# BioinformaticsToolsmith/MeShClust

Measured on AMD Instinct MI355X. Metric: sequences clustered/sec (+ NW cell-updates/sec) at 1/2/4/8 MI355X, higher is better.
Workload: dtype u8

## Files before the change

### include/meshclust_amd.h

```cpp
#ifndef MESHCLUST_AMD_H
#define MESHCLUST_AMD_H

#include <stddef.h>
#include <stdint.h>

#ifdef __cplusplus
extern "C" {
#endif

#define MC_ABI_VERSION 1

#define MC_OK 0
#define MC_ERR_ARG 1
#define MC_ERR_HIP 2
#define MC_ERR_STATE 3
#define MC_ERR_OOM 4
#define MC_ERR_INPUT 5
#define MC_ERR_UNSUPPORTED 6
#define MC_ERR_TIMEOUT 7

#define MC_FEAT_ALIGN (1 << 0)
#define MC_FEAT_LD (1 << 1)
#define MC_FEAT_MANHATTAN (1 << 2)
#define MC_FEAT_INTERSECTION (1 << 4)
// ... 86 lines not shown
int mc_orient_pairs(mc_ctx *ctx, const uint32_t *a, const uint32_t *b, uint64_t m, uint8_t *strand ,
                    uint64_t *sad );

#define MC_ASSIGN_MAX_TOP 8
int mc_assign_top(mc_ctx *ctx, const uint32_t *centre_ids, uint32_t C, const uint32_t *query_ids, uint64_t M,
                  double sim, int strands , uint32_t K ,
                  uint32_t *hit , double *hit_val , uint8_t *hit_strand ,
                  uint32_t *n_similar , uint64_t *stats );

int mc_nw_identity(mc_ctx *ctx, const uint32_t *a, const uint32_t *b, uint64_t m, double *ident,
                   int32_t *len, int32_t *ids);

int mc_nw_identity_raw(mc_ctx *ctx, const uint8_t *a, const uint64_t *a_off, const uint8_t *b,
                       const uint64_t *b_off, uint64_t m, double *ident, int32_t *len,
                       int32_t *ids, int32_t *score);

int mc_revcomp_sequences(mc_ctx *ctx, const uint32_t *ids, uint64_t m, uint8_t *bytes, uint64_t *off);

#define MC_IDENT_BATCH_PAIRS (1ull << 20)
#define MC_IDENT_BATCH_BYTES (256ull << 20)
int mc_nw_identity_strands(mc_ctx *ctx, const uint32_t *a, const uint32_t *b, const uint8_t *a_minus, uint64_t m,
                           double *ident, int32_t *len, int32_t *ids);

#define MC_CIGAR_I 1u
#define MC_CIGAR_D 2u
#define MC_CIGAR_EQ 7u
#define MC_CIGAR_X 8u
#define MC_ALIGN_BATCH_PAIRS (1ull << 16)
#define MC_ALIGN_SCRATCH_BYTES (1ull << 30)
int mc_nw_align_strands(mc_ctx *ctx, const uint32_t *a, const uint32_t *b, const uint8_t *a_minus, uint64_t m,
                        uint32_t *cigar, uint64_t cap, uint64_t *cig_off ,
                        int32_t *score, int32_t *len, int32_t *ids);
int mc_nw_align_profile(mc_ctx *ctx, double *out , int reset);

int mc_set_align_band(mc_ctx *ctx, int mode );
int mc_nw_band_plan(mc_ctx *ctx, const uint32_t *a, const uint32_t *b, const uint8_t *a_minus, uint64_t m,
                    int32_t *w , int32_t *score );
int mc_nw_band_profile(mc_ctx *ctx, double *out , int reset);

#define MC_PILEUP_CH 8
int mc_nw_pileup_strands(mc_ctx *ctx, const uint32_t *a, const uint32_t *b, const uint8_t *a_minus, uint64_t m,
                         const uint32_t *targets, uint32_t nt, uint64_t *row_off ,
                         uint32_t *table , uint64_t cap_rows,
                         int32_t *score, int32_t *len, int32_t *ids );
int mc_nw_pileup_profile(mc_ctx *ctx, double *out , int reset);

// ... 89 lines not shown
```

### meshclust_amd/__init__.py

```python
import ctypes as C
import os
import subprocess

import numpy as np

HERE = os.path.dirname(os.path.abspath(__file__))
ROOT = os.path.dirname(HERE)
LIB_DIR = os.path.join(HERE, "lib")
BIN = os.path.join(HERE, "bin", "meshclust")
GPU_LIB = os.environ.get("MC_GPU_LIB", os.path.join(LIB_DIR, "libmcgpu.so"))
HOST_LIB = os.path.join(LIB_DIR, "libmeshclust.so")
HEADER = os.path.join(ROOT, "include", "meshclust_amd.h")

FEAT_ALIGN, FEAT_LD, FEAT_MANHATTAN = 1, 2, 4
FEAT_INTERSECTION, FEAT_PEARSON, FEAT_KULCZYNSKI2 = 16, 32, 1024
COMBO_SQUARED, COMBO_SELF = 1, 2
ASSIGN_NONE = 0xFFFFFFFF
MC_STRAND_PLUS, MC_STRAND_MINUS = 1, 2
ASSIGN_MAX_TOP = 8
ERR_ARG, ERR_UNSUPPORTED = 1, 6
ERR_STATE = 3
CIGAR_I, CIGAR_D, CIGAR_EQ, CIGAR_X = 1, 2, 7, 8
PILEUP_CH = 8
MSA_GAP = ord("-")
MSA_CH = 8
QUAL_MAX = 93
FAMILIES = ("kmer", "keys", "pairs", "scan", "finalize", "mean_shift", "nw", "layout")


class MCError(RuntimeError):
    pass


def build(jobs=8):
    subprocess.run(["make", "-s", "-j%d" % jobs, "-C", os.path.join(HERE, "csrc")], check=True)


class Classifier(C.Structure):
    _fields_ = [
        ("n_single", C.c_int32),
        ("lookup", C.c_uint16 * 8),
        ("is_sim", C.c_int32 * 8),
        ("mins", C.c_double * 8),
        ("maxs", C.c_double * 8),
        ("n_combo", C.c_int32),
        ("combo_kind", C.c_int32 * 8),
        ("combo_len", C.c_int32 * 8),
        ("combo_idx", (C.c_int32 * 4) * 8),
        ("weights", C.c_double * 9),
# ... 19 lines not shown


def _p(a):
    return a.ctypes.data_as(C.c_void_p) if a is not None else None


def gpu_lib():
    global _gpu
    if _gpu is None:
        if not os.path.exists(GPU_LIB):
            raise ImportError("libmcgpu.so not built (run meshclust_amd.build()); no CPU fallback exists")
        lib = C.CDLL(GPU_LIB)
        lib.mc_last_error.restype = C.c_char_p
        lib.mc_ctx_create.argtypes = [C.c_int, C.POINTER(C.c_void_p)]
        lib.mc_ctx_destroy.argtypes = [C.c_void_p]
        for name in ("mc_load_sequences", "mc_load_packed", "mc_kmer_max", "mc_kmer_build", "mc_get_histograms", "mc_distance_keys",
                     "mc_pair_features", "mc_set_classifier", "mc_classify_pairs", "mc_nw_identity",
                     "mc_nw_identity_raw", "mc_set_order", "mc_kill", "mc_cluster_begin", "mc_scan",
                     "mc_mean_shift", "mc_update_iteration", "mc_timers", "mc_classify_values", "mc_mean_shift_select", "mc_accumulate",
                     "mc_scan_part", "mc_scan_commit", "mc_comm_unique_id", "mc_comm_create", "mc_comm_allgather",
                     "mc_comm_stats", "mc_comm_destroy", "mc_sync", "mc_assign", "mc_assign_strands",
                     "mc_revcomp_rows", "mc_assign_top", "mc_revcomp_sequences", "mc_nw_identity_strands",
                     "mc_nw_align_strands", "mc_nw_align_profile", "mc_nw_pileup_strands", "mc_nw_pileup_profile",
                     "mc_kmer_max_strands", "mc_kmer_build_strands", "mc_orient_pairs"):
            getattr(lib, name).restype = C.c_int
        lib.mc_comm_create.argtypes = [C.c_int, C.c_int, C.c_int, C.c_char_p, C.POINTER(C.c_void_p)]
        lib.mc_comm_allgather.argtypes = [C.c_void_p, C.c_void_p, C.c_uint64, C.c_void_p]
        lib.mc_comm_stats.argtypes = [C.c_void_p, C.POINTER(C.c_uint64), C.POINTER(C.c_uint64)]
        lib.mc_comm_destroy.argtypes = [C.c_void_p, C.c_int]
        lib.mc_assign.argtypes = [C.c_void_p, C.c_void_p, C.c_uint32, C.c_void_p, C.c_uint64, C.c_double,
                                  C.c_void_p, C.c_void_p, C.c_void_p, C.c_void_p]
        lib.mc_assign_strands.argtypes = [C.c_void_p, C.c_void_p, C.c_uint32, C.c_void_p, C.c_uint64, C.c_double, C.c_int,
                                          C.c_void_p, C.c_void_p, C.c_void_p, C.c_void_p, C.c_void_p]
        lib.mc_revcomp_rows.argtypes = [C.c_void_p, C.c_void_p, C.c_uint64, C.c_void_p]
        lib.mc_assign_top.argtypes = [C.c_void_p, C.c_void_p, C.c_uint32, C.c_void_p, C.c_uint64, C.c_double, C.c_int,
                                      C.c_uint32, C.c_void_p, C.c_void_p, C.c_void_p, C.c_void_p, C.c_void_p]
        lib.mc_revcomp_sequences.argtypes = [C.c_void_p, C.c_void_p, C.c_uint64, C.c_void_p, C.c_void_p]
        lib.mc_nw_identity_strands.argtypes = [C.c_void_p, C.c_void_p, C.c_void_p, C.c_void_p, C.c_uint64, C.c_void_p,
                                               C.c_void_p, C.c_void_p]
        lib.mc_nw_align_strands.argtypes = [C.c_void_p, C.c_void_p, C.c_void_p, C.c_void_p, C.c_uint64, C.c_void_p,
                                            C.c_uint64, C.c_void_p, C.c_void_p, C.c_void_p, C.c_void_p]
        lib.mc_nw_align_profile.argtypes = [C.c_void_p, C.c_void_p, C.c_int]
        lib.mc_nw_pileup_strands.argtypes = [C.c_void_p, C.c_void_p, C.c_void_p, C.c_void_p, C.c_uint64, C.c_void_p, C.c_uint32,
                                             C.c_void_p, C.c_void_p, C.c_uint64, C.c_void_p, C.c_void_p, C.c_void_p]
        lib.mc_nw_pileup_profile.argtypes = [C.c_void_p, C.c_void_p, C.c_int]
        lib.mc_kmer_max_strands.argtypes = [C.c_void_p, C.c_int, C.c_int, C.POINTER(C.c_uint64)]
        lib.mc_kmer_build_strands.argtypes = [C.c_void_p, C.c_int, C.c_int, C.c_int]
        lib.mc_orient_pairs.argtypes = [C.c_void_p, C.c_void_p, C.c_void_p, C.c_uint64, C.c_void_p, C.c_void_p]
        lib.mc_load_qualities.restype = C.c_int
        lib.mc_load_qualities.argtypes = [C.c_void_p, C.c_void_p, C.c_uint64]
        lib.mc_nw_qpileup_strands.restype = C.c_int
        lib.mc_nw_qpileup_strands.argtypes = [C.c_void_p, C.c_void_p, C.c_void_p, C.c_void_p, C.c_uint64, C.c_void_p, C.c_uint32,
                                              C.c_void_p, C.c_void_p, C.c_void_p, C.c_uint64, C.c_void_p, C.c_void_p, C.c_void_p]
        for name in ("mc_nw_msa_begin", "mc_nw_msa_rows", "mc_nw_msa_end", "mc_nw_msa_profile"):
            getattr(lib, name).restype = C.c_int
        lib.mc_nw_msa_begin.argtypes = [C.c_void_p, C.c_void_p, C.c_void_p, C.c_void_p, C.c_uint64, C.c_void_p, C.c_uint32,
                                        C.c_void_p, C.c_void_p, C.c_void_p, C.c_void_p, C.c_void_p, C.c_void_p]
        lib.mc_nw_msa_rows.argtypes = [C.c_void_p, C.c_uint64, C.c_uint64, C.c_void_p, C.c_uint64, C.c_void_p]
        lib.mc_nw_msa_end.argtypes = [C.c_void_p]
        lib.mc_nw_msa_profile.argtypes = [C.c_void_p, C.c_void_p, C.c_int]
        lib.mc_nw_msa_counts.restype = C.c_int
        lib.mc_nw_msa_counts.argtypes = [C.c_void_p, C.c_uint32, C.c_uint32, C.c_void_p, C.c_void_p, C.c_void_p, C.c_uint64]
# ... 404 lines not shown
        self._ck(self.lib.mc_nw_identity(self.ctx, _p(a), _p(b), C.c_uint64(len(a)), _p(ident), _p(ln), _p(ids)),
               "mc_nw_identity")
        return ident, ln, ids

    def revcomp_sequences(self, ids):
        ids = np.ascontiguousarray(ids, np.uint32)
        off = np.zeros(len(ids) + 1, np.uint64)
        self._ck(self.lib.mc_revcomp_sequences(self.ctx, _p(ids), len(ids), None, _p(off)), "mc_revcomp_sequences")
        out = np.zeros(int(off[-1]), np.uint8)
        self._ck(self.lib.mc_revcomp_sequences(self.ctx, _p(ids), len(ids), _p(out), _p(off)), "mc_revcomp_sequences")
        return out, off

    def nw_identity_strands(self, a, b, a_minus=None):
        a = np.ascontiguousarray(a, np.uint32)
        b = np.ascontiguousarray(b, np.uint32)
        am = None if a_minus is None else np.ascontiguousarray(a_minus, np.uint8)
        assert am is None or len(am) == len(a)
        ident = np.zeros(len(a))
        ln = np.zeros(len(a), np.int32)
        ids = np.zeros(len(a), np.int32)
        self._ck(self.lib.mc_nw_identity_strands(self.ctx, _p(a), _p(b), _p(am), C.c_uint64(len(a)), _p(ident), _p(ln),
                                               _p(ids)), "mc_nw_identity_strands")
        return ident, ln, ids

    def nw_align_strands(self, a, b, a_minus=None, cigar=True):
        a = np.ascontiguousarray(a, np.uint32)
        b = np.ascontiguousarray(b, np.uint32)
        am = None if a_minus is None else np.ascontiguousarray(a_minus, np.uint8)
        assert len(b) == len(a) and (am is None or len(am) == len(a))
        m = len(a)
        off = np.zeros(m + 1, np.uint64)
        sc = np.zeros(m, np.int32)
        ln = np.zeros(m, np.int32)
        ids = np.zeros(m, np.int32)
        if not cigar:
            self._ck(self.lib.mc_nw_align_strands(self.ctx, _p(a), _p(b), _p(am), C.c_uint64(m), None, C.c_uint64(0), _p(off),
                                                _p(sc), _p(ln), _p(ids)), "mc_nw_align_strands")
            return None, off, sc, ln, ids
        cap = 0
        for x in (a, b):
            self._ck(self.lib.mc_revcomp_sequences(self.ctx, _p(x), m, None, _p(off)), "mc_revcomp_sequences")
            cap += int(off[-1])
        words = np.zeros(cap, np.uint32)
        self._ck(self.lib.mc_nw_align_strands(self.ctx, _p(a), _p(b), _p(am), C.c_uint64(m), _p(words), C.c_uint64(cap), _p(off),
                                            _p(sc), _p(ln), _p(ids)), "mc_nw_align_strands")
        return words[:int(off[-1])], off, sc, ln, ids
# ... 274 lines not shown
        seg = arr(ptr[2], C.c_int32, 2 * int(seg_off[-1])).copy()
        out = []
        for i in range(n):
            s = seg[2 * int(seg_off[i]):2 * int(seg_off[i + 1])]
            out.append((self.lib.mcl_header(self.h, i).decode(), codes[int(seq_off[i]):int(seq_off[i + 1])],
                        [[int(s[j]), int(s[j + 1])] for j in range(0, len(s), 2)]))
        return out

    def label_identities(self, engine, a, b, both_strands=False):
        a = np.ascontiguousarray(a, np.uint32)
        b = np.ascontiguousarray(b, np.uint32)
        assert len(a) == len(b)
        out = np.zeros(len(a))
        err = C.create_string_buffer(1024)
        self.lib.mcl_label_identities.restype = C.c_int
        self.lib.mcl_label_identities.argtypes = [C.c_void_p, C.c_void_p, C.c_void_p, C.c_void_p, C.c_uint64, C.c_int,
                                                  C.c_void_p, C.c_char_p, C.c_int]
        rc = self.lib.mcl_label_identities(self.h, engine.ctx, _p(a), _p(b), len(a), 1 if both_strands else 0, _p(out),
                                           err, 1024)
        if rc != 0:
            raise MCError("mcl_label_identities failed (%d): %s" % (rc, err.value.decode()))
        return out

    def run(self, engine, args=(), upload=True, clstr=None, comm=None):
        import json
        argv = [b"meshclust"] + [a.encode() for a in args]
        arr = (C.c_char_p * len(argv))(*argv)
        buf = C.create_string_buffer(1 << 16)
        if comm is not None:
            rc = self.lib.mcl_run_sharded(self.h, engine.ctx, len(argv), arr, 1 if upload else 0,
                                          clstr.encode() if clstr else None, buf, len(buf), comm.rank, comm.world,
                                          C.cast(comm.callback, C.c_void_p), comm.user)
        else:
            rc = self.lib.mcl_run(self.h, engine.ctx, len(argv), arr, 1 if upload else 0,
                                  clstr.encode() if clstr else None, buf, len(buf))
        st = json.loads(buf.value.decode() or "{}")
        if rc != 0 or "error" in st:
            raise MCError("mcl_run failed (%d): %s" % (rc, st))
        if upload:
            engine.n = self.n
        engine.width, engine.B = st.get("width", engine.width), 4 ** st["k"] if "k" in st else engine.B
        return st

    def __del__(self):
        try:
            self.lib.mcl_free(self.h)
# ... 3 lines not shown
```

### meshclust_amd/csrc/host/capi.cpp

```cpp
#include <chrono>
#include <cstring>
#include <string>
#include <vector>

#include "runner.hpp"

extern "C" {

static void *parse_entry(const char *const *files, int nfiles, int threads, bool keep_qual, char *err, int errcap) {
  auto ds = std::make_unique<mc::Dataset>();
  try {
    std::vector<std::string> f(files, files + nfiles);
    mc::parse_fasta_files(f, *ds, threads > 0 ? threads : 1, keep_qual);
    return ds.release();
  } catch (const std::exception &e) {
    if (err && errcap > 0) snprintf(err, errcap, "%s", e.what());
    return nullptr;
  }
}

void *mcl_parse(const char *const *files, int nfiles, int threads, char *err, int errcap) {
  return parse_entry(files, nfiles, threads, false, err, errcap);
}

void *mcl_parse_q(const char *const *files, int nfiles, int threads, char *err, int errcap) {
  return parse_entry(files, nfiles, threads, true, err, errcap);
}
// ... 75 lines not shown
  try {
    mc::TrainerConfig tc;
    tc.both_strands = both_strands != 0;
    mc::PhaseTimer timer;
    mc::Trainer tr(*ds, ctx, tc, timer);
    std::vector<mc::PairId> pairs(m);
    for (uint64_t i = 0; i < m; i++) {
      if (a[i] >= ds->size() || b[i] >= ds->size()) throw mc::Error("pair id out of range", 1);
      pairs[i] = mc::PairId(a[i], b[i]);
    }
    std::vector<double> id;
    tr.nw_batch(pairs, id);
    for (uint64_t i = 0; i < m; i++) ident[i] = id[i];
    return 0;
  } catch (const mc::Error &e) {
    if (err && errcap > 0) snprintf(err, errcap, "%s", e.what());
    return e.code ? e.code : 1;
  } catch (const std::exception &e) {
    if (err && errcap > 0) snprintf(err, errcap, "%s", e.what());
    return 1;
  }
}

int mcl_run(void *dsv, mc_ctx *ctx, int argc, char **argv, int upload, const char *clstr_path, char *stats,
            int cap) {
  return run_common(dsv, ctx, argc, argv, upload, clstr_path, stats, cap, nullptr);
}

int mcl_run_sharded(void *dsv, mc_ctx *ctx, int argc, char **argv, int upload, const char *clstr_path, char *stats,
                    int cap, int rank, int world, int (*allgather)(void *, const void *, uint64_t, void *),
                    void *user) {
  if (world < 1 || rank < 0 || rank >= world || (world > 1 && !allgather)) return 1;
  mc::ShardComm comm;
  comm.rank = rank;
  comm.world = world;
  comm.allgather = allgather;
  comm.user = user;
  return run_common(dsv, ctx, argc, argv, upload, clstr_path, stats, cap, &comm);
}
}
```

### meshclust_amd/csrc/host/cluster.hpp

```cpp
#pragma once
#include <cstddef>
#include <cstdint>
#include <string>
#include <vector>

#include "bvec.hpp"
#include "common.hpp"
#include "fasta.hpp"

namespace mc {

struct Center {
  uint32_t centre;
  std::vector<uint32_t> points;
  bool del = false;
};


void fault_point(const ShardComm *comm, const char *stage);

struct ClusterConfig {
  const ShardComm *comm = nullptr;
  double sim = 0.90;
  int iterations = 15;
  int delta = 5;
  bool verbose = true;
  bool align = false;
  int width = 1;
};

struct ClusterStats {
  uint64_t scan_steps = 0;
  uint64_t scan_candidates = 0;
  uint64_t update_evals = 0;
  uint64_t merge_evals = 0;
  uint64_t update_iters_fixed = 0;
  uint64_t update_evals_run = 0;
  uint64_t nw_pairs = 0, nw_cells = 0;
  uint64_t align_nw_pairs = 0, align_nw_cells = 0;
  std::string accum_path;
  std::string update_path;
};

std::vector<Center> mean_shift_cluster(const Dataset &ds, mc_ctx *ctx, BVec &bv, const ClusterConfig &cfg,
                                       PhaseTimer &timer, ClusterStats &stats);

void write_clstr(const std::string &path, const Dataset &ds, const std::vector<Center> &part, int threads = 1);

}
```

### meshclust_amd/csrc/host/common.hpp

```cpp
#pragma once
#include <chrono>
#include <cstdint>
#include <cstdio>
#include <cstdlib>
#include <map>
#include <stdexcept>
#include <string>
#include <vector>

#include "../../../include/meshclust_amd.h"

extern "C" {
int mc_kmer_max_strands(mc_ctx *, int, int, uint64_t *) __attribute__((weak));
int mc_kmer_build_strands(mc_ctx *, int, int, int) __attribute__((weak));
int mc_orient_pairs(mc_ctx *, const uint32_t *, const uint32_t *, uint64_t, uint8_t *, uint64_t *) __attribute__((weak));
int mc_nw_identity_strands(mc_ctx *, const uint32_t *, const uint32_t *, const uint8_t *, uint64_t, double *, int32_t *,
                           int32_t *) __attribute__((weak));
}

namespace mc {

struct Error : std::runtime_error {
  int code;
  explicit Error(const std::string &m, int c = 1) : std::runtime_error(m), code(c) {}
};
struct ShardComm {
  int rank = 0, world = 1;
  int (*allgather)(void *user, const void *in, uint64_t bytes, void *out) = nullptr;
  void *user = nullptr;
};

struct PeerError : Error {
  explicit PeerError(const std::string &m) : Error(m, 1) {}
};

void comm_phase(const ShardComm *comm, const char *phase);

inline void check(int rc, const char *what) {
  if (rc != MC_OK) {
    const char *e = mc_last_error();
// ... 47 lines not shown
```

### meshclust_amd/csrc/host/runner.cpp

```cpp
#include "runner.hpp"

#include "model.hpp"

#include <libgen.h>
#include <malloc.h>
#include <sys/stat.h>
#include <unistd.h>

#include <algorithm>
#include <cerrno>
#include <chrono>
#include <cmath>
#include <atomic>
#include <condition_variable>
#include <exception>
#include <mutex>
#include <memory>
#include <thread>
#include <cstdio>
#include <cstdlib>
#include <cstring>
#include <limits>

#ifdef _OPENMP
// ... 318 lines not shown
    bvec_thread.join();
  }
  fault_point(comm, "train");
  rr.timer.add("bvec.overlapped", bvec_ms);
  rr.timer.add("bvec.overlapped.insert", bvec_lap[0]);
  rr.timer.add("bvec.overlapped.finalize", bvec_lap[1]);
  if (bvec_err) std::rethrow_exception(bvec_err);
  mc_classifier cls = tr.classifier();
  check(mc_set_classifier(ctx, &cls), "mc_set_classifier");
  rr.cls = cls;
  rr.similarity = opt.similarity;
  rr.align = opt.align;
  ClusterConfig cc;
  cc.sim = opt.similarity;
  cc.iterations = opt.iterations;
  cc.delta = opt.delta;
  cc.verbose = verbose;
  cc.align = opt.align;
  cc.width = rr.width;
  cc.comm = comm;
  rr.part = mean_shift_cluster(ds, ctx, *bvp, cc, rr.timer, rr.stats);
  rr.stats.nw_pairs = tr.nw_pairs;
  rr.stats.nw_cells = tr.nw_cells;
  if (opt.both_strands) {
    Scope s(rr.timer, "orient");
    std::vector<uint32_t> a, b;
    for (const Center &c : rr.part)
      for (uint32_t p : c.points) {
        a.push_back(p);
        b.push_back(c.centre);
      }
    std::vector<uint8_t> st(a.size(), 0);
    std::vector<uint64_t> sad(2 * a.size(), 0);
    check(mc_orient_pairs(ctx, a.data(), b.data(), a.size(), st.data(), sad.data()), "mc_orient_pairs");
    size_t at = 0;
    for (const Center &c : rr.part) {
      rr.member_strand.emplace_back(st.begin() + at, st.begin() + at + c.points.size());
      rr.member_sad.emplace_back(sad.begin() + 2 * at, sad.begin() + 2 * (at + c.points.size()));
      at += c.points.size();
    }
    for (uint8_t v : st) rr.members_minus += v;
  }
  rr.timer.add("total_pipeline",
               std::chrono::duration<double, std::milli>(std::chrono::steady_clock::now() - t0).count());
  return rr;
}

std::string stats_json(const RunResult &rr, double parse_ms, double write_ms) {
  char b[512];
  std::string o;
  snprintf(b, sizeof b, "{\"n\": %zu, \"k\": %d, \"width\": %d, \"clusters\": %zu, \"parse_ms\": %.3f, \"write_ms\": %.3f",
           rr.n, rr.k, rr.width, rr.part.size(), parse_ms, write_ms);
  o += b;
  snprintf(b, sizeof b,
           ", \"scan_steps\": %llu, \"scan_candidates\": %llu, \"update_evals\": %llu, \"merge_evals\": %llu"
           ", \"nw_pairs\": %llu, \"nw_cells\": %llu, \"align_nw_pairs\": %llu, \"align_nw_cells\": %llu",
           (unsigned long long)rr.stats.scan_steps, (unsigned long long)rr.stats.scan_candidates,
           (unsigned long long)rr.stats.update_evals, (unsigned long long)rr.stats.merge_evals,
           (unsigned long long)rr.stats.nw_pairs, (unsigned long long)rr.stats.nw_cells,
           (unsigned long long)rr.stats.align_nw_pairs, (unsigned long long)rr.stats.align_nw_cells);
  o += b;
  if (rr.strands != 1) {
    snprintf(b, sizeof b, ", \"strands\": %d, \"k_auto_length\": %llu, \"members_minus\": %llu", rr.strands,
             (unsigned long long)rr.k_auto_length, (unsigned long long)rr.members_minus);
    o += b;
  }
  o += ", \"accum_path\": \"" + rr.stats.accum_path + "\"";
  if (!rr.stats.update_path.empty()) o += ", \"update_path\": \"" + rr.stats.update_path + "\"";
  o += ", \"update_iters_fixed\": " + std::to_string(rr.stats.update_iters_fixed);
  o += ", \"update_evals_run\": " + std::to_string(rr.stats.update_evals_run);
  o += ", \"phases_ms\": {";
  for (size_t i = 0; i < rr.timer.order.size(); i++) {
    snprintf(b, sizeof b, "%s\"%s\": %.3f", i ? ", " : "", rr.timer.order[i].c_str(), rr.timer.ms.at(rr.timer.order[i]));
    o += b;
  }
  o += "}}";
  return o;
}

void save_model_files(const Options &opt, const Dataset &ds, const RunResult &rr) {
  if (!opt.save_model.empty()) {
    Model m;
// ... 207 lines not shown
```

### meshclust_amd/csrc/host/trainer.cpp

```cpp
#include "trainer.hpp"

#include "lazysort.hpp"

#include <algorithm>
#include <array>
#include <atomic>
#include <cmath>
#include <cstdio>
#include <cstring>
#include <exception>
#include <memory>
#include <set>
#include <thread>

namespace mc {

namespace {

struct ExitZero : Error {
  ExitZero(const std::string &m) : Error(m, 0) {}
};

inline int get_bin(double x, double min_align, double max_align, int num_bins) {
  if (x >= max_align) return num_bins - 1;
  if (x <= min_align) return 0;
// ... 57 lines not shown
  if (pairs.empty()) return;
  for (const auto &p : pairs) {
    nw_pairs++;
    nw_cells += ds_.lengths[p.first] * ds_.lengths[p.second];
  }
  if (!cfg_.both_strands) {
    check(mc_nw_identity(ctx_, a.data(), b.data(), pairs.size(), ident.data(), nullptr, nullptr), "mc_nw_identity");
    return;
  }
  strands_engine_check();
  const size_t m = pairs.size();
  for (const auto &p : pairs) {
    nw_pairs++;
    nw_cells += ds_.lengths[p.first] * ds_.lengths[p.second];
  }
  a.insert(a.end(), a.begin(), a.begin() + m);
  b.insert(b.end(), b.begin(), b.begin() + m);
  std::vector<uint8_t> minus(2 * m, 0);
  std::fill(minus.begin() + m, minus.end(), 1);
  std::vector<double> both(2 * m, 0.0);
  check(mc_nw_identity_strands(ctx_, a.data(), b.data(), minus.data(), 2 * m, both.data(), nullptr, nullptr),
        "mc_nw_identity_strands");
  for (size_t i = 0; i < m; i++) ident[i] = both[m + i] > both[i] ? both[m + i] : both[i];
}

namespace {
struct HdrKey {
  uint64_t k0, k1;
  uint32_t len, id;
};
HdrKey hdr_key(const Dataset &ds, uint32_t id) {
  const std::string_view h = ds.headers[id];
  unsigned char b[16] = {0};
  memcpy(b, h.data(), h.size() < 16 ? h.size() : 16);
  uint64_t w0 = 0, w1 = 0;
  for (int i = 0; i < 8; i++) {
    w0 = (w0 << 8) | b[i];
    w1 = (w1 << 8) | b[8 + i];
  }
  return HdrKey{w0, w1, (uint32_t)std::min<size_t>(h.size(), 0xffffffffu), id};
}
int hdr_cmp(const Dataset &ds, const HdrKey &x, const HdrKey &y) {
  if (x.k0 != y.k0) return x.k0 < y.k0 ? -1 : 1;
  if (x.k1 != y.k1) return x.k1 < y.k1 ? -1 : 1;
  if (x.len <= 16 && y.len <= 16) return x.len < y.len ? -1 : x.len > y.len ? 1 : 0;
  const int c = ds.headers[x.id].compare(ds.headers[y.id]);
// ... 62 lines not shown
    else points = length_order(ds_, cfg_.threads);
    uint32_t begin_pt = points[N / 2];
    std::vector<uint16_t> key0(N);
    check(mc_distance_keys(ctx_, &begin_pt, 1, all_ids.data(), N, key0.data()), "mc_distance_keys");
    for (size_t t = 0; t < N; t++) w[t] = ((uint64_t)key0[points[t]] << 32) | points[t];
    exact_sort(w);
    for (size_t t = 0; t < N; t++) points[t] = (uint32_t)w[t];
  }
  int num_iterations = (int)std::ceil(((double)cfg_.n_points) / cfg_.max_pts_from_one) - 1;
  if (num_iterations <= 0) throw Error("sample size must exceed points per pivot (integer division by zero in Trainer::split)", 1);
  std::vector<uint32_t> indices;
  for (int i = 0; i <= num_iterations; i++) indices.push_back(points[(size_t)i * (N - 1) / (size_t)num_iterations]);
  if (cfg_.verbose) printf("Point pairs: %zu\n", indices.size());
  const size_t to_add_each = cfg_.max_pts_from_one / 2;
  const size_t P = indices.size();
  const bool long_reads = [&] {
    uint64_t tot = 0;
    for (size_t t = 0; t < N; t++) tot += ds_.lengths[t];
    return N > 0 && tot / N > 4096;
  }();
  const int look = [&] {
    const char *e = getenv("MC_NW_LOOKAHEAD");
    const int v = e ? atoi(e) : long_reads ? 1 : 2;
    return v < 1 ? 1 : v > 4 ? 4 : v;
  }();
  const bool spine = [&] {
    const char *e = getenv("MC_NW_SPINE");
    if (e) return atoi(e) != 0;
    return N > 0 && !long_reads;
  }();
  struct Plan {
    std::vector<size_t> pos;
    std::vector<std::array<int, 2>> kid;
  };
  auto tree = [&](size_t p, size_t o, int d, Plan &pl) {
    pl.pos.clear();
    pl.kid.clear();
    if (o == 0) return;
    std::vector<size_t> off;
    pl.pos.push_back(p);
    pl.kid.push_back({-1, -1});
    off.push_back(o);
    std::vector<int> level = {0};
    for (int l = 1; l < d; l++) {
      std::vector<int> next;
      for (int n : level) {
        const size_t oc = off[(size_t)n] / 2;
        if (oc == 0) continue;
        for (int side = 0; side < 2; side++) {
          pl.kid[(size_t)n][(size_t)side] = (int)pl.pos.size();
          next.push_back((int)pl.pos.size());
          pl.pos.push_back(side ? pl.pos[(size_t)n] + off[(size_t)n] : pl.pos[(size_t)n] - off[(size_t)n]);
          pl.kid.push_back({-1, -1});
          off.push_back(oc);
        }
      }
      level.swap(next);
    }
  };
  const int W = cfg_.comm && cfg_.comm->world > 1 ? cfg_.comm->world : 1;
  const size_t per = (P + (size_t)W - 1) / (size_t)W;
  const size_t i0 = std::min(P, per * (size_t)(W > 1 ? cfg_.comm->rank : 0)), i1 = std::min(P, i0 + per);
  const int spine_levels = [&] {
    const char *e = getenv("MC_NW_SPINE_LEVELS");
    const int v = e ? atoi(e) : 0;
    if (v > 0) return v;
    const size_t chains = i1 > i0 ? i1 - i0 : 1;
    return (int)std::max<size_t>(1, 2048 / chains);
  }();
  auto left_spine = [&](size_t p, size_t o, Plan &pl) {
    pl.pos.clear();
    pl.kid.clear();
    for (int lv = 0; o > 0 && lv < spine_levels; o /= 2, lv++) {
      if (!pl.pos.empty()) pl.kid.back()[0] = (int)pl.pos.size();
      pl.pos.push_back(p);
      pl.kid.push_back({-1, -1});
      p -= o;
    }
  };
  const uint64_t nw_pairs0 = nw_pairs, nw_cells0 = nw_cells;
  {
    Scope s(timer_, "train.sort_keys");
    Scope s3(timer_, "train.sort_keys.pivots");
    if (i1 > i0) check(mc_split_begin(ctx_, indices.data() + i0, (uint32_t)(i1 - i0), points.data(), N), "mc_split_begin");
  }
  std::vector<uint32_t> q_arr, q_ids;
  std::vector<uint64_t> q_pos;
  auto select = [&]() {
    q_ids.resize(q_arr.size());
    if (!q_arr.empty()) {
      std::vector<uint32_t> la(q_arr.size());
      for (size_t q = 0; q < q_arr.size(); q++) la[q] = q_arr[q] - (uint32_t)i0;
      check(mc_split_select(ctx_, q_arr.size(), la.data(), q_pos.data(), q_ids.data()), "mc_split_select");
    }
  };
  std::vector<size_t> offset(P, N / 4), pivot(P, 2 * (N / 4));
  std::vector<char> active(P, 1);
  auto sample_positions = [&](size_t pv, std::vector<size_t> &out) {
    const size_t npts = N;
    double before_inc = (double)pv / to_add_each, after_inc = ((double)(npts - pv)) / to_add_each;
    double bs = 0, as = (double)pv;
    for (int t = 0; t < (int)to_add_each; t++, bs += before_inc) out.push_back((size_t)(int)std::round(bs));
    for (int t = 0; t < (int)to_add_each && std::round(as) < (double)npts; t++, as += after_inc)
      out.push_back((size_t)(int)std::round(as));
  };
  {
    Scope s(timer_, "train.nw_search");
    std::vector<PairId> batch;
    std::vector<size_t> who, first;
    std::vector<Plan> plan(P);
    for (int round = 0;; round++) {
      who.clear();
      for (size_t i = i0; i < i1; i++) {
        if (active[i] && offset[i] == 0) active[i] = 0;
        if (active[i]) who.push_back(i);
      }
      {
        Scope s2(timer_, "train.nw_search.resolve");
        first.assign(who.size() + 1, 0);
        q_arr.clear();
        q_pos.clear();
        for (size_t t = 0; t < who.size(); t++) {
          const size_t i = who[t];
          if (round == 0 && spine) left_spine(pivot[i], offset[i], plan[i]);
          else tree(pivot[i], offset[i], look, plan[i]);
          for (size_t n = 0; n < plan[i].pos.size(); n++) {
            q_arr.push_back((uint32_t)i);
            q_pos.push_back(plan[i].pos[n]);
          }
          first[t + 1] = q_arr.size();
        }
        select();
        batch.resize(q_arr.size());
        for (size_t q = 0; q < q_arr.size(); q++) batch[q] = PairId(indices[q_arr[q]], q_ids[q]);
      }
      if (batch.empty()) break;
      std::vector<double> al;
      {
        Scope s3(timer_, "train.nw_search.align");
        nw_batch(batch, al);
      }
      for (size_t t = 0; t < who.size(); t++) {
        const size_t i = who[t];
        const double *val = al.data() + first[t];
        for (int n = 0; n >= 0 && active[i];) {
          const double algn = val[n];
          if (algn < cfg_.cutoff) {
            pivot[i] -= offset[i];
            n = plan[i].kid[(size_t)n][0];
          } else if (algn > cfg_.cutoff) {
            pivot[i] += offset[i];
            n = plan[i].kid[(size_t)n][1];
          } else {
            active[i] = 0;
            break;
          }
          offset[i] /= 2;
          if (offset[i] == 0) break;
        }
      }
    }
  }
  int aerr = 0;
  std::vector<std::vector<PairId>> bufs(P);
  {
    Scope sb(timer_, "train.sample");
    q_arr.clear();
    q_pos.clear();
    std::vector<size_t> sp;
    for (size_t i = i0; i < i1; i++) {
      sp.clear();
      sample_positions(pivot[i], sp);
      for (size_t x : sp) {
        q_arr.push_back((uint32_t)i);
        q_pos.push_back(x);
      }
    }
    select();
    for (size_t q = 0; q < q_arr.size(); q++) {
      const uint32_t p = indices[q_arr[q]], x = q_ids[q];
      bufs[q_arr[q]].push_back(hdr_less(p, x) ? PairId(p, x) : PairId(x, p));
    }
    if (i1 > i0) check(mc_split_end(ctx_), "mc_split_end");
    const size_t cap = per * (2 * to_add_each);
    std::vector<uint64_t> mine(3 + per + cap, 0), all;
    mine[0] = nw_pairs - nw_pairs0;
    mine[1] = nw_cells - nw_cells0;
    size_t np = 0;
    for (size_t i = i0; i < i1; i++) {
      mine[3 + (i - i0)] = pivot[i];
      for (const PairId &pr : bufs[i]) mine[3 + per + np++] = ((uint64_t)pr.first << 32) | pr.second;
    }
    mine[2] = np;
    if (gather(mine, all)) {
      nw_pairs = nw_pairs0;
      nw_cells = nw_cells0;
      for (int r = 0; r < W; r++) {
        const uint64_t *b = all.data() + (size_t)r * mine.size();
        const size_t r0 = std::min(P, per * (size_t)r), r1 = std::min(P, r0 + per);
        nw_pairs += b[0];
        nw_cells += b[1];
        for (size_t i = r0; i < r1; i++) {
          pivot[i] = b[3 + (i - r0)];
          if (r != cfg_.comm->rank) bufs[i].clear();
        }
        if (r == cfg_.comm->rank) continue;
        for (uint64_t q = 0; q < b[2] && r1 > r0; q++)
          bufs[r0].push_back(PairId((uint32_t)(b[3 + per + q] >> 32), (uint32_t)b[3 + per + q]));
      }
    }
  }
  Scope sp(timer_, "train.sample.pair_set");
  for (size_t i = 0; i < P; i++) {
    double before_inc = (double)pivot[i] / to_add_each;
    double after_inc = ((double)(N - pivot[i])) / to_add_each;
    if (before_inc < 1) aerr = 1;
    else if (after_inc < 1) aerr = -1;
    pairs.insert(pairs.end(), bufs[i].begin(), bufs[i].end());
  }
  {
    const std::vector<uint32_t> ord = header_set_order(ds_, pairs.size(), [&](size_t i) { return pairs[i]; });
    std::vector<PairId> set(ord.size());
    for (size_t i = 0; i < ord.size(); i++) set[i] = pairs[ord[i]];
    pairs.swap(set);
  }
  if (aerr < 0) fprintf(stderr, "Warning: Alignment may be too small for sampling\n");
  else if (aerr > 0) fprintf(stderr, "Warning: Alignment may be too large for sampling\n");
  return pairs;
}

void Trainer::get_labels(const std::vector<PairId> &vec, std::vector<Labeled> &bp, std::vector<Labeled> &bn) {
// ... 167 lines not shown
```

### meshclust_amd/csrc/host/trainer.hpp

```cpp
#pragma once
#include <cstddef>
#include <cstdint>
#include <utility>
#include <vector>

#include "common.hpp"
#include "fasta.hpp"
#include "feature.hpp"
#include "glm.hpp"

namespace mc {

using PairId = std::pair<uint32_t, uint32_t>;

struct TrainerConfig {
  size_t n_points = 3000;
  size_t max_pts_from_one = 20;
  double cutoff = 0.90;
  int k = 4;
  int threads = 1;
  bool verbose = true;
  const ShardComm *comm = nullptr;
  std::vector<uint32_t> length_order;
  bool both_strands = false;
};

class Trainer {
 public:
  Trainer(const Dataset &ds, mc_ctx *ctx, const TrainerConfig &cfg, PhaseTimer &timer)
      : ds_(ds), ctx_(ctx), cfg_(cfg), timer_(timer) {}
  void train(double acc_cutoff = 97.5);
  static std::vector<uint32_t> length_order(const Dataset &ds, int threads);
  mc_classifier classifier() const { return feat.to_classifier(weights); }
  void nw_batch(const std::vector<PairId> &pairs, std::vector<double> &ident);

  FeatureSet feat;
  std::vector<double> weights;
  std::vector<PairId> split_pairs;
  std::vector<std::pair<PairId, double>> label_pos, label_neg;
  uint64_t nw_pairs = 0, nw_cells = 0;

 private:
  std::vector<PairId> split();
  void get_labels(const std::vector<PairId> &vec, std::vector<std::pair<PairId, double>> &bp,
                  std::vector<std::pair<PairId, double>> &bn);
  Matrix feat_matrix(const std::vector<PairId> &pos, const std::vector<PairId> &neg, int ncols,
                     Matrix &labels);
  bool gather(const std::vector<uint64_t> &mine, std::vector<uint64_t> &all) const;
  bool hdr_less(uint32_t a, uint32_t b) const;

  const Dataset &ds_;
  mc_ctx *ctx_;
  TrainerConfig cfg_;
  PhaseTimer &timer_;
};

}
```

Before: 2.761 million.

## Add q-gram lemma screen to skip NW alignments in trainer pivot search

Adds a GPU q-gram counting kernel, with a host fallback, that computes shared q-grams per pair. The q-gram lemma then marks pairs as certainly below the identity cutoff, so their Needleman-Wunsch alignment is skipped during the trainer's binary pivot search. The search plan is also restructured: a spine round decides whether screening is decisive, which enables deeper lookahead and speculative pruning of subtrees. This trades extra kernel launches and more complex search bookkeeping for fewer expensive NW alignments, and it only pays off when many candidates fall below the cutoff.

```diff
diff --git a/include/meshclust_amd.h b/include/meshclust_amd.h
--- a/include/meshclust_amd.h
+++ b/include/meshclust_amd.h
@@ -132,6 +132,10 @@
 int mc_nw_identity_strands(mc_ctx *ctx, const uint32_t *a, const uint32_t *b, const uint8_t *a_minus, uint64_t m,
                            double *ident, int32_t *len, int32_t *ids);
 
+#define MC_QGRAM_NA 0xffffffffu
+int mc_qgram_common(mc_ctx *ctx, const uint32_t *a, const uint32_t *b, const uint8_t *a_minus, uint64_t m, int q,
+                    uint32_t *common);
+
 #define MC_CIGAR_I 1u
 #define MC_CIGAR_D 2u
 #define MC_CIGAR_EQ 7u
diff --git a/meshclust_amd/__init__.py b/meshclust_amd/__init__.py
--- a/meshclust_amd/__init__.py
+++ b/meshclust_amd/__init__.py
@@ -25,6 +25,7 @@
 MSA_GAP = ord("-")
 MSA_CH = 8
 QUAL_MAX = 93
+QGRAM_NA = 0xFFFFFFFF
 FAMILIES = ("kmer", "keys", "pairs", "scan", "finalize", "mean_shift", "nw", "layout")
 
 
@@ -90,7 +91,7 @@
                      "mc_comm_stats", "mc_comm_destroy", "mc_sync", "mc_assign", "mc_assign_strands",
                      "mc_revcomp_rows", "mc_assign_top", "mc_revcomp_sequences", "mc_nw_identity_strands",
                      "mc_nw_align_strands", "mc_nw_align_profile", "mc_nw_pileup_strands", "mc_nw_pileup_profile",
-                     "mc_kmer_max_strands", "mc_kmer_build_strands", "mc_orient_pairs"):
+                     "mc_kmer_max_strands", "mc_kmer_build_strands", "mc_orient_pairs", "mc_qgram_common"):
             getattr(lib, name).restype = C.c_int
         lib.mc_comm_create.argtypes = [C.c_int, C.c_int, C.c_int, C.c_char_p, C.POINTER(C.c_void_p)]
         lib.mc_comm_allgather.argtypes = [C.c_void_p, C.c_void_p, C.c_uint64, C.c_void_p]
@@ -106,6 +107,7 @@
         lib.mc_revcomp_sequences.argtypes = [C.c_void_p, C.c_void_p, C.c_uint64, C.c_void_p, C.c_void_p]
         lib.mc_nw_identity_strands.argtypes = [C.c_void_p, C.c_void_p, C.c_void_p, C.c_void_p, C.c_uint64, C.c_void_p,
                                                C.c_void_p, C.c_void_p]
+        lib.mc_qgram_common.argtypes = [C.c_void_p, C.c_void_p, C.c_void_p, C.c_void_p, C.c_uint64, C.c_int, C.c_void_p]
         lib.mc_nw_align_strands.argtypes = [C.c_void_p, C.c_void_p, C.c_void_p, C.c_void_p, C.c_uint64, C.c_void_p,
                                             C.c_uint64, C.c_void_p, C.c_void_p, C.c_void_p, C.c_void_p]
         lib.mc_nw_align_profile.argtypes = [C.c_void_p, C.c_void_p, C.c_int]
@@ -556,6 +558,15 @@
         self._ck(self.lib.mc_nw_identity_strands(self.ctx, _p(a), _p(b), _p(am), C.c_uint64(len(a)), _p(ident), _p(ln),
                                                _p(ids)), "mc_nw_identity_strands")
         return ident, ln, ids
+
+    def qgram_common(self, a, b, q, a_minus=None):
+        a = np.ascontiguousarray(a, np.uint32)
+        b = np.ascontiguousarray(b, np.uint32)
+        am = None if a_minus is None else np.ascontiguousarray(a_minus, np.uint8)
+        assert len(a) == len(b) and (am is None or len(am) == len(a))
+        out = np.zeros(len(a), np.uint32)
+        self._ck(self.lib.mc_qgram_common(self.ctx, _p(a), _p(b), _p(am), C.c_uint64(len(a)), int(q), _p(out)), "mc_qgram_common")
+        return out
 
     def nw_align_strands(self, a, b, a_minus=None, cigar=True):
         a = np.ascontiguousarray(a, np.uint32)
@@ -876,6 +887,18 @@
             raise MCError("mcl_label_identities failed (%d): %s" % (rc, err.value.decode()))
         return out
 
+    def qscreen_common(self, a, b, q, a_minus=None):
+        a = np.ascontiguousarray(a, np.uint32)
+        b = np.ascontiguousarray(b, np.uint32)
+        am = None if a_minus is None else np.ascontiguousarray(a_minus, np.uint8)
+        assert len(a) == len(b) and (am is None or len(am) == len(a))
+        out = np.zeros(len(a), np.uint32)
+        self.lib.mcl_qscreen_common.restype = C.c_int
+        self.lib.mcl_qscreen_common.argtypes = [C.c_void_p, C.c_void_p, C.c_void_p, C.c_void_p, C.c_uint64, C.c_int, C.c_void_p]
+        if self.lib.mcl_qscreen_common(self.h, _p(a), _p(b), _p(am), len(a), int(q), _p(out)) != 0:
+            raise MCError("mcl_qscreen_common: pair id out of range")
+        return out
+
     def run(self, engine, args=(), upload=True, clstr=None, comm=None):
         import json
         argv = [b"meshclust"] + [a.encode() for a in args]
diff --git a/meshclust_amd/csrc/gpu/qgram.hip b/meshclust_amd/csrc/gpu/qgram.hip
--- /dev/null
+++ b/meshclust_amd/csrc/gpu/qgram.hip
@@ -0,0 +1,114 @@
+#include <algorithm>
+
+#include "abi_util.hpp"
+#include "mcgpu.hpp"
+
+namespace mcg {
+
+namespace {
+
+constexpr int NT = 256;
+constexpr int QMAX = 7;
+constexpr uint32_t NA = 0xffffffffu;
+
+__device__ __forceinline__ uint32_t gram_at(const uint32_t *__restrict__ w, uint32_t j, int q, uint32_t mask) {
+  const uint32_t wi = j >> 4, sh = 2 * (j & 15);
+  uint64_t v = w[wi];
+  if (sh + 2 * (uint32_t)q > 32) v |= (uint64_t)w[wi + 1] << 32;
+  return (uint32_t)(v >> sh) & mask;
+}
+
+__device__ __forceinline__ uint32_t revcomp_gram(uint32_t g, int q, uint32_t mask) {
+  const uint32_t y = __brev(~g & mask);
+  return (((y & 0x55555555u) << 1) | ((y >> 1) & 0x55555555u)) >> (32 - 2 * q);
+}
+
+__global__ __launch_bounds__(NT) void qgram_kernel(const uint32_t *__restrict__ packed, const uint64_t *__restrict__ pk_off,
+                                                   const uint64_t *__restrict__ seq_off, const uint8_t *__restrict__ impure,
+                                                   const uint32_t *__restrict__ a, const uint32_t *__restrict__ b,
+                                                   const uint8_t *__restrict__ a_minus, uint32_t m, int q,
+                                                   uint32_t *__restrict__ common) {
+  __shared__ uint32_t tab[1 << (2 * QMAX)];
+  const uint32_t mask = (1u << (2 * q)) - 1, nbin = 1u << (2 * q);
+  for (uint32_t p = blockIdx.x; p < m; p += gridDim.x) {
+    const uint32_t ia = a[p], ib = b[p];
+    const uint64_t la = seq_off[ia + 1] - seq_off[ia], lb = seq_off[ib + 1] - seq_off[ib];
+    if (la < (uint64_t)q || lb < (uint64_t)q || impure[ia] || impure[ib]) {
+      if (threadIdx.x == 0) common[p] = NA;
+      continue;
+    }
+    const bool minus = a_minus && a_minus[p];
+    for (uint32_t t = threadIdx.x; t < nbin; t += NT) tab[t] = 0;
+    __syncthreads();
+    const uint32_t *wa = packed + pk_off[ia], *wb = packed + pk_off[ib];
+    const uint32_t na = (uint32_t)la - (uint32_t)q + 1, nb = (uint32_t)lb - (uint32_t)q + 1;
+    for (uint32_t j = threadIdx.x; j < na; j += NT) {
+      const uint32_t g = gram_at(wa, j, q, mask);
+      atomicAdd(&tab[minus ? revcomp_gram(g, q, mask) : g], 1u);
+    }
+    __syncthreads();
+    uint32_t hits = 0;
+    for (uint32_t j = threadIdx.x; j < nb; j += NT) {
+      uint32_t *e = &tab[gram_at(wb, j, q, mask)];
+      if ((int32_t)atomicSub(e, 1u) > 0) hits++;
+      else atomicAdd(e, 1u);
+    }
+    for (int o = 32; o > 0; o >>= 1) hits += __shfl_down(hits, o, 64);
+    __syncthreads();
+    if ((threadIdx.x & 63) == 0) tab[threadIdx.x >> 6] = hits;
+    __syncthreads();
+    if (threadIdx.x == 0) common[p] = tab[0] + tab[1] + tab[2] + tab[3];
+    __syncthreads();
+  }
+}
+
+}
+
+static int launch_qgram(mc_ctx *c, const uint32_t *d_a, const uint32_t *d_b, const uint8_t *d_minus, uint32_t m, int q,
+                        uint32_t *d_common) {
+  const unsigned grid = std::min<uint32_t>(m, 1u << 16);
+  timed_begin(c);
+  qgram_kernel<<<grid, NT, 0, c->stream>>>((const uint32_t *)c->packed.p, (const uint64_t *)c->pk_off.p,
+                                           (const uint64_t *)c->seq_off.p, (const uint8_t *)c->impure.p, d_a, d_b, d_minus, m, q,
+                                           d_common);
+  timed_end(c, F_PAIRS);
+  MCG_CHECK(hipGetLastError());
+  return MC_OK;
+}
+
+}
+
+using namespace mcg;
+
+extern "C" int mc_qgram_common(mc_ctx *c, const uint32_t *a, const uint32_t *b, const uint8_t *a_minus, uint64_t m, int q,
+                               uint32_t *common) {
+  if (!c || !c->codes.p) return MC_ERR_STATE;
+  if (m == 0) return MC_OK;
+  if (!a || !b || !common) return MC_ERR_ARG;
+  if (q < 1 || q > QMAX) {
+    set_error("mc_qgram_common: q must be in 1..7");
+    return MC_ERR_ARG;
+  }
+  MCG_CHECK(hipSetDevice(c->device));
+  TRY(check_ids(c, a, m));
+  TRY(check_ids(c, b, m));
+  for (uint64_t i = 0; i < m; i++)
+    for (uint32_t id : {a[i], b[i]})
+      if (c->h_seq_off[id + 1] - c->h_seq_off[id] >= (1ull << 31)) {
+        set_error("mc_qgram_common: a read of 2^31 bases or more");
+        return MC_ERR_UNSUPPORTED;
+      }
+  constexpr uint64_t CHUNK = 1u << 20;
+  for (uint64_t i0 = 0; i0 < m; i0 += CHUNK) {
+    const uint64_t mb = std::min(CHUNK, m - i0);
+    TRY(upload(c, c->s_d, a + i0, mb, c->stream));
+    TRY(upload(c, c->s_e, b + i0, mb, c->stream));
+    if (a_minus) TRY(upload(c, c->s_g, a_minus + i0, mb, c->stream));
+    TRY(ensure(c->s_f, mb * 4 + 64));
+    TRY(launch_qgram(c, (const uint32_t *)c->s_d.p, (const uint32_t *)c->s_e.p, a_minus ? (const uint8_t *)c->s_g.p : nullptr,
+                     (uint32_t)mb, q, (uint32_t *)c->s_f.p));
+    TRY(download_parts(c, {{common + i0, c->s_f.p, mb * 4}}, c->stream));
+  }
+  flush_timers(c);
+  return MC_OK;
+}
diff --git a/meshclust_amd/csrc/host/capi.cpp b/meshclust_amd/csrc/host/capi.cpp
--- a/meshclust_amd/csrc/host/capi.cpp
+++ b/meshclust_amd/csrc/host/capi.cpp
@@ -3,6 +3,7 @@
 #include <string>
 #include <vector>
 
+#include "qscreen.hpp"
 #include "runner.hpp"
 
 extern "C" {
@@ -124,6 +125,15 @@
   }
 }
 
+int mcl_qscreen_common(void *dsv, const uint32_t *a, const uint32_t *b, const uint8_t *a_minus, uint64_t m, int q,
+                       uint32_t *common) {
+  const auto *ds = (const mc::Dataset *)dsv;
+  for (uint64_t i = 0; i < m; i++)
+    if (a[i] >= ds->size() || b[i] >= ds->size()) return 1;
+  for (uint64_t i = 0; i < m; i++) common[i] = mc::qscreen::common(*ds, a[i], b[i], a_minus && a_minus[i], q);
+  return 0;
+}
+
 int mcl_run(void *dsv, mc_ctx *ctx, int argc, char **argv, int upload, const char *clstr_path, char *stats,
             int cap) {
   return run_common(dsv, ctx, argc, argv, upload, clstr_path, stats, cap, nullptr);
diff --git a/meshclust_amd/csrc/host/cluster.hpp b/meshclust_amd/csrc/host/cluster.hpp
--- a/meshclust_amd/csrc/host/cluster.hpp
+++ b/meshclust_amd/csrc/host/cluster.hpp
@@ -37,6 +37,7 @@
   uint64_t update_iters_fixed = 0;
   uint64_t update_evals_run = 0;
   uint64_t nw_pairs = 0, nw_cells = 0;
+  uint64_t nw_screened = 0;
   uint64_t align_nw_pairs = 0, align_nw_cells = 0;
   std::string accum_path;
   std::string update_path;
diff --git a/meshclust_amd/csrc/host/common.hpp b/meshclust_amd/csrc/host/common.hpp
--- a/meshclust_amd/csrc/host/common.hpp
+++ b/meshclust_amd/csrc/host/common.hpp
@@ -16,6 +16,7 @@
 int mc_orient_pairs(mc_ctx *, const uint32_t *, const uint32_t *, uint64_t, uint8_t *, uint64_t *) __attribute__((weak));
 int mc_nw_identity_strands(mc_ctx *, const uint32_t *, const uint32_t *, const uint8_t *, uint64_t, double *, int32_t *,
                            int32_t *) __attribute__((weak));
+int mc_qgram_common(mc_ctx *, const uint32_t *, const uint32_t *, const uint8_t *, uint64_t, int, uint32_t *) __attribute__((weak));
 }
 
 namespace mc {
diff --git a/meshclust_amd/csrc/host/qscreen.hpp b/meshclust_amd/csrc/host/qscreen.hpp
--- /dev/null
+++ b/meshclust_amd/csrc/host/qscreen.hpp
@@ -0,0 +1,66 @@
+#pragma once
+#include <algorithm>
+#include <cstdint>
+#include <vector>
+
+#include "fasta.hpp"
+
+namespace mc {
+namespace qscreen {
+
+constexpr uint32_t NA = 0xffffffffu;
+constexpr int QMAX = 7, QMIN = 4;
+
+inline int pick_q(double c) {
+  for (int q = QMAX; q >= QMIN; q--)
+    if ((double)q * (1.0 - c) <= 0.75) return q;
+  return 0;
+}
+
+inline bool below(uint32_t C, uint64_t la, uint64_t lb, double c, int q) {
+  return C != NA && (double)((uint64_t)C + (uint64_t)q + 2) <= (1.0 - (double)q * (1.0 - c)) * (double)std::max(la, lb);
+}
+
+inline bool pure(const Dataset &ds, uint32_t i) {
+  const uint64_t s = ds.seq_off[i], e = ds.seq_off[i + 1];
+  const auto it = std::lower_bound(ds.exc_pos.begin(), ds.exc_pos.end(), s);
+  if (it != ds.exc_pos.end() && *it < e) return false;
+  uint64_t covered = 0;
+  for (uint64_t g = ds.seg_off[i]; g < ds.seg_off[i + 1]; g++) covered += (uint64_t)(ds.seg[2 * g + 1] - ds.seg[2 * g] + 1);
+  return covered == e - s;
+}
+
+template <typename F>
+inline void grams(const Dataset &ds, uint32_t i, bool minus, int q, F f) {
+  const uint64_t len = ds.seq_off[i + 1] - ds.seq_off[i];
+  const uint32_t *w = ds.packed.data() + ds.pk_off[i];
+  const uint32_t mask = (1u << (2 * q)) - 1;
+  uint32_t fw = 0, rc = 0;
+  for (uint64_t j = 0; j < len; j++) {
+    const uint32_t d = (w[j >> 4] >> (2 * (j & 15))) & 3u;
+    fw = (fw >> 2) | (d << (2 * (q - 1)));
+    rc = ((rc << 2) | (3u - d)) & mask;
+    if (j + 1 >= (uint64_t)q) f(minus ? rc : fw);
+  }
+}
+
+inline uint32_t common(const Dataset &ds, uint32_t a, uint32_t b, bool minus, int q) {
+  if (q < 1 || q > QMAX) return NA;
+  const uint64_t la = ds.seq_off[a + 1] - ds.seq_off[a], lb = ds.seq_off[b + 1] - ds.seq_off[b];
+  if (la < (uint64_t)q || lb < (uint64_t)q || !pure(ds, a) || !pure(ds, b)) return NA;
+  static thread_local std::vector<uint32_t> occ;
+  occ.resize((size_t)1 << (2 * QMAX), 0);
+  grams(ds, a, minus, q, [&](uint32_t g) { occ[g]++; });
+  uint32_t c = 0;
+  grams(ds, b, false, q, [&](uint32_t g) {
+    if (occ[g]) {
+      occ[g]--;
+      c++;
+    }
+  });
+  grams(ds, a, minus, q, [&](uint32_t g) { occ[g] = 0; });
+  return c;
+}
+
+}
+}
diff --git a/meshclust_amd/csrc/host/runner.cpp b/meshclust_amd/csrc/host/runner.cpp
--- a/meshclust_amd/csrc/host/runner.cpp
+++ b/meshclust_amd/csrc/host/runner.cpp
@@ -364,6 +364,7 @@
   rr.part = mean_shift_cluster(ds, ctx, *bvp, cc, rr.timer, rr.stats);
   rr.stats.nw_pairs = tr.nw_pairs;
   rr.stats.nw_cells = tr.nw_cells;
+  rr.stats.nw_screened = tr.nw_screened;
   if (opt.both_strands) {
     Scope s(rr.timer, "orient");
     std::vector<uint32_t> a, b;
@@ -396,10 +397,10 @@
   o += b;
   snprintf(b, sizeof b,
            ", \"scan_steps\": %llu, \"scan_candidates\": %llu, \"update_evals\": %llu, \"merge_evals\": %llu"
-           ", \"nw_pairs\": %llu, \"nw_cells\": %llu, \"align_nw_pairs\": %llu, \"align_nw_cells\": %llu",
+           ", \"nw_pairs\": %llu, \"nw_cells\": %llu, \"nw_screened\": %llu, \"align_nw_pairs\": %llu, \"align_nw_cells\": %llu",
            (unsigned long long)rr.stats.scan_steps, (unsigned long long)rr.stats.scan_candidates,
            (unsigned long long)rr.stats.update_evals, (unsigned long long)rr.stats.merge_evals,
-           (unsigned long long)rr.stats.nw_pairs, (unsigned long long)rr.stats.nw_cells,
+           (unsigned long long)rr.stats.nw_pairs, (unsigned long long)rr.stats.nw_cells, (unsigned long long)rr.stats.nw_screened,
            (unsigned long long)rr.stats.align_nw_pairs, (unsigned long long)rr.stats.align_nw_cells);
   o += b;
   if (rr.strands != 1) {
diff --git a/meshclust_amd/csrc/host/trainer.cpp b/meshclust_amd/csrc/host/trainer.cpp
--- a/meshclust_amd/csrc/host/trainer.cpp
+++ b/meshclust_amd/csrc/host/trainer.cpp
@@ -1,6 +1,7 @@
 #include "trainer.hpp"
 
 #include "lazysort.hpp"
+#include "qscreen.hpp"
 
 #include <algorithm>
 #include <array>
@@ -104,6 +105,30 @@
   check(mc_nw_identity_strands(ctx_, a.data(), b.data(), minus.data(), 2 * m, both.data(), nullptr, nullptr),
         "mc_nw_identity_strands");
   for (size_t i = 0; i < m; i++) ident[i] = both[m + i] > both[i] ? both[m + i] : both[i];
+}
+
+void Trainer::screen(const std::vector<PairId> &pairs, int q, bool host, std::vector<char> &out) {
+  const size_t m = pairs.size(), S = cfg_.both_strands ? 2 : 1;
+  out.assign(m, 0);
+  if (m == 0) return;
+  std::vector<uint32_t> cnt(S * m, qscreen::NA);
+  if (host) {
+#pragma omp parallel for schedule(static) num_threads(cfg_.threads)
+    for (size_t j = 0; j < S * m; j++) cnt[j] = qscreen::common(ds_, pairs[j % m].first, pairs[j % m].second, j >= m, q);
+  } else {
+    std::vector<uint32_t> a(S * m), b(S * m);
+    std::vector<uint8_t> minus(S * m, 0);
+    for (size_t j = 0; j < S * m; j++) {
+      a[j] = pairs[j % m].first;
+      b[j] = pairs[j % m].second;
+      minus[j] = j >= m;
+    }
+    check(mc_qgram_common(ctx_, a.data(), b.data(), S == 2 ? minus.data() : nullptr, S * m, q, cnt.data()), "mc_qgram_common");
+  }
+  for (size_t i = 0; i < m; i++) {
+    const uint64_t la = ds_.lengths[pairs[i].first], lb = ds_.lengths[pairs[i].second];
+    out[i] = qscreen::below(cnt[i], la, lb, cfg_.cutoff, q) && (S == 1 || qscreen::below(cnt[m + i], la, lb, cfg_.cutoff, q));
+  }
 }
 
 namespace {
@@ -212,7 +237,7 @@
   const int look = [&] {
     const char *e = getenv("MC_NW_LOOKAHEAD");
     const int v = e ? atoi(e) : long_reads ? 1 : 2;
-    return v < 1 ? 1 : v > 4 ? 4 : v;
+    return v < 1 ? 1 : v > 7 ? 7 : v;
   }();
   const bool spine = [&] {
     const char *e = getenv("MC_NW_SPINE");
@@ -251,13 +276,33 @@
   const int W = cfg_.comm && cfg_.comm->world > 1 ? cfg_.comm->world : 1;
   const size_t per = (P + (size_t)W - 1) / (size_t)W;
   const size_t i0 = std::min(P, per * (size_t)(W > 1 ? cfg_.comm->rank : 0)), i1 = std::min(P, i0 + per);
+  const int screen_q = [&] {
+    const char *e = getenv("MC_NW_SCREEN");
+    if (e && !strcmp(e, "0")) return 0;
+    return qscreen::pick_q(cfg_.cutoff);
+  }();
+  const bool screen_host = [&] {
+    const char *e = getenv("MC_NW_SCREEN");
+    return !mc_qgram_common || (e && !strcmp(e, "host"));
+  }();
+  const int spine_gen = (int)std::max<size_t>(1, 2048 / (i1 > i0 ? i1 - i0 : 1));
   const int spine_levels = [&] {
     const char *e = getenv("MC_NW_SPINE_LEVELS");
     const int v = e ? atoi(e) : 0;
-    if (v > 0) return v;
-    const size_t chains = i1 > i0 ? i1 - i0 : 1;
-    return (int)std::max<size_t>(1, 2048 / chains);
-  }();
+    return v > 0 ? v : screen_q ? 64 : spine_gen;
+  }();
+  const int spine_align = [&] {
+    const char *e = getenv("MC_NW_SPINE_ALIGN");
+    const int v = e ? atoi(e) : 0;
+    return v > 0 ? v : spine_gen;
+  }();
+  const bool screen_spine = screen_q && !(getenv("MC_NW_SPINE") && atoi(getenv("MC_NW_SPINE")) == 0);
+  const int look_deep = [&] {
+    const char *e = getenv("MC_NW_LOOKAHEAD");
+    return e || long_reads ? look : 5;
+  }();
+  const bool speculate = !(getenv("MC_NW_SPECULATE") && atoi(getenv("MC_NW_SPECULATE")) == 0);
+  bool decisive = false;
   auto left_spine = [&](size_t p, size_t o, Plan &pl) {
     pl.pos.clear();
     pl.kid.clear();
@@ -268,7 +313,7 @@
       p -= o;
     }
   };
-  const uint64_t nw_pairs0 = nw_pairs, nw_cells0 = nw_cells;
+  const uint64_t nw_pairs0 = nw_pairs, nw_cells0 = nw_cells, nw_screened0 = nw_screened;
   {
     Scope s(timer_, "train.sort_keys");
     Scope s3(timer_, "train.sort_keys.pivots");
@@ -296,8 +341,10 @@
   };
   {
     Scope s(timer_, "train.nw_search");
-    std::vector<PairId> batch;
+    std::vector<PairId> planned, batch;
     std::vector<size_t> who, first;
+    std::vector<char> scr;
+    std::vector<int> slot;
     std::vector<Plan> plan(P);
     for (int round = 0;; round++) {
       who.clear();
@@ -305,6 +352,7 @@
         if (active[i] && offset[i] == 0) active[i] = 0;
         if (active[i]) who.push_back(i);
       }
+      const bool spine_round = round == 0 && (spine || screen_spine);
       {
         Scope s2(timer_, "train.nw_search.resolve");
         first.assign(who.size() + 1, 0);
@@ -312,8 +360,8 @@
         q_pos.clear();
         for (size_t t = 0; t < who.size(); t++) {
           const size_t i = who[t];
-          if (round == 0 && spine) left_spine(pivot[i], offset[i], plan[i]);
-          else tree(pivot[i], offset[i], look, plan[i]);
+          if (spine_round) left_spine(pivot[i], offset[i], plan[i]);
+          else tree(pivot[i], offset[i], decisive ? look_deep : look, plan[i]);
           for (size_t n = 0; n < plan[i].pos.size(); n++) {
             q_arr.push_back((uint32_t)i);
             q_pos.push_back(plan[i].pos[n]);
@@ -321,21 +369,57 @@
           first[t + 1] = q_arr.size();
         }
         select();
-        batch.resize(q_arr.size());
-        for (size_t q = 0; q < q_arr.size(); q++) batch[q] = PairId(indices[q_arr[q]], q_ids[q]);
-      }
-      if (batch.empty()) break;
+        planned.resize(q_arr.size());
+        for (size_t q = 0; q < q_arr.size(); q++) planned[q] = PairId(indices[q_arr[q]], q_ids[q]);
+      }
+      if (planned.empty()) break;
+      {
+        Scope s4(timer_, "train.nw_search.screen");
+        scr.assign(planned.size(), 0);
+        if (screen_q) screen(planned, screen_q, screen_host, scr);
+        if (spine_round) {
+          size_t roots = 0;
+          for (size_t t = 0; t < who.size(); t++) roots += first[t + 1] > first[t] && scr[first[t]];
+          decisive = 2 * roots >= who.size() && roots > 0;
+        }
+        const int round_cap = !spine_round ? 1 << 30 : decisive || !spine ? 0 : spine_align;
+        slot.assign(planned.size(), -1);
+        batch.clear();
+        std::vector<char> need;
+        for (size_t t = 0; t < who.size(); t++) {
+          const Plan &pl = plan[who[t]];
+          const size_t f = first[t];
+          need.assign(pl.pos.size(), 0);
+          need[0] = 1;
+          int aligned = 0;
+          for (size_t n = 0; n < pl.pos.size(); n++) {
+            if (!need[n]) continue;
+            if (scr[f + n]) {
+              nw_screened++;
+              if (pl.kid[n][0] >= 0) need[(size_t)pl.kid[n][0]] = 1;
+              continue;
+            }
+            if (aligned >= round_cap) continue;
+            aligned++;
+            slot[f + n] = (int)batch.size();
+            batch.push_back(planned[f + n]);
+            for (int side = decisive && speculate ? 1 : 0; side < 2; side++)
+              if (pl.kid[n][(size_t)side] >= 0) need[(size_t)pl.kid[n][(size_t)side]] = 1;
+          }
+        }
+      }
       std::vector<double> al;
-      {
+      if (!batch.empty()) {
         Scope s3(timer_, "train.nw_search.align");
         nw_batch(batch, al);
       }
       for (size_t t = 0; t < who.size(); t++) {
-        const size_t i = who[t];
-        const double *val = al.data() + first[t];
+        const size_t i = who[t], f = first[t];
         for (int n = 0; n >= 0 && active[i];) {
-          const double algn = val[n];
-          if (algn < cfg_.cutoff) {
+          const bool below = scr[f + (size_t)n];
+          if (!below && slot[f + (size_t)n] < 0) break;
+          const double algn = below ? 0.0 : al[(size_t)slot[f + (size_t)n]];
+          if (below || algn < cfg_.cutoff) {
             pivot[i] -= offset[i];
             n = plan[i].kid[(size_t)n][0];
           } else if (algn > cfg_.cutoff) {
@@ -372,31 +456,34 @@
       bufs[q_arr[q]].push_back(hdr_less(p, x) ? PairId(p, x) : PairId(x, p));
     }
     if (i1 > i0) check(mc_split_end(ctx_), "mc_split_end");
-    const size_t cap = per * (2 * to_add_each);
-    std::vector<uint64_t> mine(3 + per + cap, 0), all;
+    const size_t cap = per * (2 * to_add_each), H = 4;
+    std::vector<uint64_t> mine(H + per + cap, 0), all;
     mine[0] = nw_pairs - nw_pairs0;
     mine[1] = nw_cells - nw_cells0;
+    mine[3] = nw_screened - nw_screened0;
     size_t np = 0;
     for (size_t i = i0; i < i1; i++) {
-      mine[3 + (i - i0)] = pivot[i];
-      for (const PairId &pr : bufs[i]) mine[3 + per + np++] = ((uint64_t)pr.first << 32) | pr.second;
+      mine[H + (i - i0)] = pivot[i];
+      for (const PairId &pr : bufs[i]) mine[H + per + np++] = ((uint64_t)pr.first << 32) | pr.second;
     }
     mine[2] = np;
     if (gather(mine, all)) {
       nw_pairs = nw_pairs0;
       nw_cells = nw_cells0;
+      nw_screened = nw_screened0;
       for (int r = 0; r < W; r++) {
         const uint64_t *b = all.data() + (size_t)r * mine.size();
         const size_t r0 = std::min(P, per * (size_t)r), r1 = std::min(P, r0 + per);
         nw_pairs += b[0];
         nw_cells += b[1];
+        nw_screened += b[3];
         for (size_t i = r0; i < r1; i++) {
-          pivot[i] = b[3 + (i - r0)];
+          pivot[i] = b[H + (i - r0)];
           if (r != cfg_.comm->rank) bufs[i].clear();
         }
         if (r == cfg_.comm->rank) continue;
         for (uint64_t q = 0; q < b[2] && r1 > r0; q++)
-          bufs[r0].push_back(PairId((uint32_t)(b[3 + per + q] >> 32), (uint32_t)b[3 + per + q]));
+          bufs[r0].push_back(PairId((uint32_t)(b[H + per + q] >> 32), (uint32_t)b[H + per + q]));
       }
     }
   }
diff --git a/meshclust_amd/csrc/host/trainer.hpp b/meshclust_amd/csrc/host/trainer.hpp
--- a/meshclust_amd/csrc/host/trainer.hpp
+++ b/meshclust_amd/csrc/host/trainer.hpp
@@ -39,6 +39,7 @@
   std::vector<PairId> split_pairs;
   std::vector<std::pair<PairId, double>> label_pos, label_neg;
   uint64_t nw_pairs = 0, nw_cells = 0;
+  uint64_t nw_screened = 0;
 
  private:
   std::vector<PairId> split();
@@ -48,6 +49,7 @@
                      Matrix &labels);
   bool gather(const std::vector<uint64_t> &mine, std::vector<uint64_t> &all) const;
   bool hdr_less(uint32_t a, uint32_t b) const;
+  void screen(const std::vector<PairId> &pairs, int q, bool host, std::vector<char> &out);
 
   const Dataset &ds_;
   mc_ctx *ctx_;
```

Result: faster. 2.886 million (median of 6 runs) (+4.5%).
